# smu-ivpl/FastInterCU-VVC

Hardware: AMD Instinct MI355X
Metric: CU-inferences/sec (batch 4096, 128x128) (higher is better)
Workload: dtype f16 (fp32 accumulate)

## Files before the change

fastintercu-vvc_amd/csrc/mlt_dispatch.cpp:

```cpp
#include "mlt_runtime.h"

const char *tuning_env(const char *name) {
  const char *e = std::getenv("MLT_TUNING");
  return (e && e[0] == '1') ? std::getenv(name) : nullptr;
}

const Tuning &tuning() {
  static const Tuning t = [] {
    auto num = [](const char *name, long dflt) { const char *e = tuning_env(name); return e ? std::atol(e) : dflt; };
    auto on = [](const char *name) { return tuning_env(name) != nullptr; };
    auto cap = [&](const char *name) { const long v = num(name, 0); return (int)(v > 0 ? v : 256); };
    Tuning u{};
    u.debug_dump_dir = tuning_env("MLT_DEBUG_DUMP_DIR");
    u.xl_kill = (int)num("MLT_XL_KILL", 0); u.xl_kill_layer = (int)num("MLT_XL_KILL_LAYER", -1);
    u.lat_pixels = num("MLT_LAT_PIXELS", 16384L);
    u.no_exact_lat = on("MLT_NO_EXACT_LAT"); u.exact_patch_big = !on("MLT_EXACT_PATCH_64K");
    u.wg_cap = cap("MLT_WG_CAP"); u.wg_cap0 = cap("MLT_WG_CAP0"); u.wg_cap1 = cap("MLT_WG_CAP1"); u.wg_cap2 = cap("MLT_WG_CAP2");
    u.l0_mfma32 = on("MLT_L0_MFMA32"); u.l1_mfma32 = !on("MLT_L1_MFMA16");
    u.no_block_fusion = on("MLT_NO_BLOCK_FUSION");
    u.no_chain = on("MLT_NO_CHAIN") || u.no_block_fusion; u.no_chain_s2 = on("MLT_NO_CHAIN_S2"); u.no_c16 = on("MLT_NO_C16"); u.chain64 = !on("MLT_NO_CHAIN64");
    u.no_l0_s5 = on("MLT_NO_L0_S5");
    u.l0_stream_min = on("MLT_NO_L0_STREAM") ? 0 : (int)num("MLT_L0_STREAM_MIN", 128);
    u.l1_stream_min = on("MLT_NO_L1_STREAM") ? 0 : (int)num("MLT_L1_STREAM_MIN", 128);
    u.guard_wait_mode = on("MLT_GUARD_SPIN_WAIT") ? 1 : on("MLT_GUARD_BLOCKING_WAIT") ? 2 : 0;
    u.no_small_mix = on("MLT_NO_SMALL_MIX"); u.no_mag_guard = on("MLT_NO_MAG_GUARD");
    u.no_graph = on("MLT_NO_GRAPH") || u.debug_dump_dir != nullptr;
    return u;
  }();
  return t;
}

namespace {

int gap_slots(int hw) { return hw >= 32 ? hw / 32 : 1; }

size_t ws_per_cu(const mlt::Model &m, int S, bool some_exact = false) {
  const int h0 = S / 2 > 0 ? S / 2 : 1;
  const int planes = (m.exact || some_exact) ? 2 : 1;
  size_t b = 4 * ((size_t)h0 * h0 * 32 * 2 * planes + 256);
  int h = S;
  for (int s = 0; s < m.n_stages; ++s) {
    h = h / 2 > 0 ? h / 2 : 1;
    b += (size_t)h * h * m.planes[s] * 2 * planes + 256;
    if (s >= 1) b += (size_t)gap_slots(h * h) * m.planes[s] * 4 + 256;
  }
  return b + 4096;
}

int ensure_ws(mlt_ctx *ctx, size_t bytes) {
  if (bytes <= ctx->ws_bytes) return MLT_OK;
  if (ctx->ws) { HIP_TRY(ctx, hipStreamSynchronize(ctx->stream)); (void)hipFree(ctx->ws); ctx->ws = nullptr; ctx->ws_bytes = 0; }
  ++ctx->ws_gen;
  HIP_TRY(ctx, hipMalloc((void **)&ctx->ws, bytes));
  ctx->ws_bytes = bytes;
  return MLT_OK;
}
}
void release_ws(mlt_ctx *ctx) {
  if (ctx->ws) { (void)hipFree(ctx->ws); ctx->ws = nullptr; ctx->ws_bytes = 0; }
  ++ctx->ws_gen;
}
namespace {

int debug_dump(mlt_ctx *ctx, const char *name, const void *dptr, size_t bytes) {
  const char *dir = tuning().debug_dump_dir;
  static int seq = 0;
  if (!dir) return MLT_OK;
  std::vector<char> host(bytes);
  HIP_TRY(ctx, hipStreamSynchronize(ctx->stream));
  HIP_TRY(ctx, hipMemcpy(host.data(), dptr, bytes, hipMemcpyDeviceToHost));
  char path[1200];
  std::snprintf(path, sizeof path, "%s/%02d_%s.bin", dir, seq++, name);
  if (FILE *f = std::fopen(path, "wb")) { std::fwrite(host.data(), 1, bytes, f); std::fclose(f); }
  return MLT_OK;
}

// ... 220 lines not shown
  a.x = x; a.y = y; a.w1 = B.conv1.d_w; a.w2 = B.conv2.d_w; a.bias1 = B.conv1.d_bias; a.bias2 = B.conv2.d_bias;
  a.w1_lo_off = B.conv1.plane_halves * 2; a.w2_lo_off = B.conv2.plane_halves * 2; a.scale1 = B.conv1.acc_scale; a.scale2 = B.conv2.acc_scale;
  a.n = n; a.h_l = ilog2(h); a.ntiles = n * (h / (w2 ? 8 : 16)) * (h / 32);
  const int wg_cap = tuning().wg_cap;
  const int grid_x = a.ntiles > wg_cap ? wg_cap : a.ntiles;
  char name[48];
  std::snprintf(name, sizeof name, "block_s1_32_h%d(conv1+conv2)", h);
  const double px = (double)n * h * h;
  Launch L{ctx};
  hipEvent_t e0 = nullptr, e1 = nullptr;
  int rc = L.prof_begin(name, 2.0 * px * 32 * 32 * 9 * 2, px * 32 * 2 * 2 + 2.0 * 18 * 1024, e0, e1, w2 ? "hi+lo weights" : "single pass");
  if (rc) return rc;
  plan_note(ctx, {{"x", x}, {"y", y}}, {{"grid", grid_x}});
  LAUNCH_TRY(ctx, mlt_launch_block32(a, w2, grid_x, ctx->stream));
  if ((rc = L.prof_end(e1))) return rc;
  return debug_dump(ctx, name, y, (size_t)px * 32 * 2);
}

int run_chain3(mlt_ctx *ctx, const mlt::Block &B0, const mlt::Block &B1, int n, int h, const void *t, const void *sc, void *y, float *gap,
               const void *s2_in, bool x_c16, bool y_c16, void *b0_hbm, bool sc_c16) {
  const int c = B0.conv2.cout;
  ChainArgs a{};
  a.x = s2_in ? s2_in : t; a.nconv = 3; a.y = y; a.gap = gap; a.n = n; a.zero = ctx->zero_page;
  a.x_c16 = x_c16 ? 1 : 0; a.y_c16 = y_c16 ? 1 : 0; a.res0_c16 = sc_c16 ? 1 : 0;
  const mlt::PackedConv *pcs[3] = {&B0.conv2, &B1.conv1, &B1.conv2};
  const bool w2 = B0.conv2.w2;
  for (int k = 0; k < 3; ++k) {
    a.cv[k].w = pcs[k]->d_w; a.cv[k].bias = pcs[k]->d_bias; a.cv[k].acc_scale = pcs[k]->acc_scale; a.cv[k].relu = 1;
    a.cv[k].w_lo_off = pcs[k]->plane_halves * 2;
    a.cv[k].lo8_scale = 0x01010101 * ((127 - pcs[k]->lo8_exp) & 0xFF);
  }
  a.cv[0].res_mode = s2_in ? 2 : 1; a.cv[0].res = sc; a.cv[0].save = 1; a.cv[2].res_mode = 2;
  if (c == 64) {
    a.cv[0].save = 0; a.cv[0].y = b0_hbm; a.cv[2].res_mode = 1; a.cv[2].res = b0_hbm;
  }
  if (s2_in) {
    const mlt::PackedConv &p2 = B0.conv1_s2c;
    a.s2_w = p2.d_w; a.s2_bias = p2.d_bias; a.s2_bias_sc = p2.d_bias_sc; a.s2_scale = p2.acc_scale;
  }
  const int hw = h * h;
  a.gap_slots = gap_slots(hw); a.gap_l = hw >= 32 ? 5 : ilog2(hw);
  const int wg_cap = tuning().wg_cap;
  const int spw = c == 256 ? 2 : 1;
  const int ntiles = (n + spw - 1) / spw;
  const int grid_x = ntiles > wg_cap ? wg_cap : ntiles;
  char name[48];
  std::snprintf(name, sizeof name, s2_in ? "stage_%d_h%d(s2+sc,conv2,conv1,conv2)" : "chain3_s1_%d_h%d(conv2+conv1+conv2)", c, h);
  const double px = (double)n * hw;
  const double flops = 3.0 * 2.0 * px * c * c * 9 + (s2_in ? 2.0 * px * c * (c / 2) * 10 : 0.0);
  const double bytes = (s2_in ? px * 4 * (c / 2) * 2 : px * c * 2 * 2) + (y ? px * c * 2 : 0.0) + 3.0 * (double)B0.conv2.w.size() * 2 +
                       (s2_in ? (double)B0.conv1_s2c.w.size() * 2 : 0.0);
  Launch L{ctx};
  hipEvent_t e0 = nullptr, e1 = nullptr;
  char variant[96];
  std::snprintf(variant, sizeof variant, "%s%s%s%s%s", w2 ? "hi+lo weights" : "single pass", x_c16 ? ", x chunk-major" : "", sc_c16 ? ", sc chunk-major" : "", y_c16 ? ", y chunk-major" : "",
                gap ? ", GAP" : "");
  int rc = L.prof_begin(name, flops, bytes, e0, e1, variant);
  if (rc) return rc;
  plan_note(ctx, {{"x", a.x}, {"sc", s2_in ? nullptr : sc}, {"y", y}, {"gap", gap}, {"b0", c == 64 ? b0_hbm : nullptr}}, {{"grid", grid_x}});
  LAUNCH_TRY(ctx, mlt_launch_chain(c, h, s2_in != nullptr, ctx->lds_oob_zero, w2, a, grid_x, ctx->stream));
  if ((rc = L.prof_end(e1))) return rc;
  if (y && (rc = debug_dump(ctx, name, y, (size_t)px * c * 2))) return rc;
  return MLT_OK;
}

int run_layer1_stream(mlt_ctx *ctx, const mlt::Block &B0, const mlt::Block &B1, int n, const void *t, const void *sc, void *y, float *gap, bool y_c16) {
  Layer1Args a{};
  a.t = t; a.sc = sc; a.y = y; a.y_c16 = y_c16 ? 1 : 0; a.gap = gap; a.gap_slots = gap_slots(32 * 32); a.n = n;
  const mlt::PackedConv *pcs[3] = {&B0.conv2, &B1.conv1, &B1.conv2};
  for (int k = 0; k < 3; ++k) { a.w[k] = pcs[k]->d_w; a.bias[k] = pcs[k]->d_bias; a.scale[k] = pcs[k]->acc_scale; }
  const int wg_cap = tuning().wg_cap1;
  const int grid_x = n > wg_cap ? wg_cap : n;
  const double px = (double)n * 32 * 32;
  Launch L{ctx};
  hipEvent_t e0 = nullptr, e1 = nullptr;
  int rc = L.prof_begin("layer1_stream_h32(conv2+conv1+conv2)", 3.0 * 2.0 * px * 64 * 64 * 9, px * 64 * 2 * 3 + 3.0 * 72 * 1024, e0, e1, y_c16 ? "single pass, y chunk-major, GAP" : "single pass, GAP");
  if (rc) return rc;
  const bool mfma32 = tuning().l1_mfma32;
  plan_note(ctx, {{"t", t}, {"sc", sc}, {"y", y}, {"gap", gap}}, {{"grid", grid_x}});
  LAUNCH_TRY(ctx, mlt_launch_layer1_stream(a, mfma32, grid_x, ctx->stream));
  if ((rc = L.prof_end(e1))) return rc;
  return debug_dump(ctx, "chain3_s1_64_h32(conv2+conv1+conv2)", y, (size_t)px * 64 * 2);
}

enum : unsigned { CLS_QUADS = 1u, CLS_FLAT = 2u, CLS_L0_STREAM = 4u, CLS_L1_STREAM = 8u, CLS_CHAIN0 = 16u  };
unsigned batch_class(const NetCfg &c, int n, const Planes &pl, bool has_flat) {
  const Tuning &tn = tuning();
  unsigned cls = 0;
  if (pl.aligned8()) cls |= CLS_QUADS;
  if (has_flat) cls |= CLS_FLAT;
  if (tn.l0_stream_min > 0 && n >= tn.l0_stream_min) cls |= CLS_L0_STREAM;
  if (tn.l1_stream_min > 0 && n >= tn.l1_stream_min) cls |= CLS_L1_STREAM;
  for (int s = 1; s < c.m->n_stages; ++s) {
    const int h = c.h_in(s), ho = h / 2 > 0 ? h / 2 : 1;
    if ((long)n * ho * ho > tn.lat_pixels) cls |= CLS_CHAIN0 << s;
  }
  return cls;
}


NetPlan plan_network(const mlt_ctx *ctx, const NetCfg &c, unsigned cls) {
  const Tuning &tn = tuning();
  const mlt::Model &m = *c.m;
  NetPlan P;
  auto add = [&](PlanStep::Kind k, int s) -> PlanStep & { PlanStep st{}; st.kind = k; st.s = (int8_t)s; P.push_back(st); return P.back(); };
  auto wants_chain = [&](int s) -> bool {
    if (s <= 0 || s >= m.n_stages || tn.no_chain || !(cls & (CLS_CHAIN0 << s))) return false;
    const mlt::Model &mm = c.model_of(s, 1);
    if (mm.exact || (mm.w2 && !ctx->lds_oob_zero)) return false;
    const int h = c.h_in(s), ho = h / 2 > 0 ? h / 2 : 1;
    const mlt::PackedConv &c2 = mm.blocks[s][0].conv2;
    const bool packing_ok = (m.planes[s] == 64 ? (c2.ct == 64 && c2.gt == 9 && tn.chain64) : (c2.ct == 128 && c2.gt == 3)) && (!mm.w2 || c2.lo8 || m.planes[s] == 64);
    return mlt_chain_supported(m.planes[s], ho) && c2.taps == 9 && c2.kc == 64 && packing_ok;
// ... 239 lines not shown
```

fastintercu-vvc_amd/csrc/mlt_kernels.h:

```cpp
#pragma once
#include <hip/hip_runtime.h>
#include <stdint.h>

#define MLT_MAX_HEADS_K 4
#define MLT_MAX_LOGITS_K 16
#define MLT_FLAT_RANGE 6
#define MLT_FLAT_EXACT_SHIFT 16

struct ConvArgs {
  const void *x;
  void *y;
  const void *w;
  const float *bias;
  const void *res;
  const void *zero;
  int n;
  int ntiles;
  int hin_l, hout_l;
  int tw_l, th_l, spw_l;
  int ph, pw, rp, half;
  uint32_t pw_magic, ph_magic, rp_magic;
  int patch_bytes;
  int relu;
  int y_c16;
// ... 57 lines not shown
  const float *bias, *bias_sc, *bias2, *bias3, *bias4;
  void *y;
  int32_t *flat;
  float acc_scale;
  int n;
  const void *w5;
  const float *bias5, *bias5_sc;
  void *y_t, *y_sc;
  float scale5;
};

#define MLT_L1_LDS_BYTES 159008
struct Layer1Args {
  const void *t;
  const void *sc;
  const void *w[3];
  const float *bias[3];
  float scale[3];
  void *y;
  int y_c16;
  float *gap;
  int gap_slots, n;
};

struct ChainConv {
  const void *w;
  size_t w_lo_off;
  int lo8_scale;
  const float *bias;
  float acc_scale;
  int relu;
  int res_mode;
  int save;
  const void *res;
  void *y;
};
struct ChainArgs {
  const void *x;
  const void *s2_w;
  const float *s2_bias, *s2_bias_sc;
  float s2_scale;
  const void *zero;
  ChainConv cv[3];
  int nconv;
  void *y;
  int y_c16;
  int x_c16;
  int res0_c16;
  float *gap;
  int gap_slots, gap_l;
  int n;
};
hipError_t mlt_launch_chain(int c, int h, bool with_s2, bool oob_zero, bool w2, const ChainArgs &a, int grid_x, hipStream_t st);
bool mlt_chain_supported(int c, int h);
hipError_t mlt_probe_lds_oob(int *d_ok, hipStream_t st);
bool mlt_stage_supported(int c, int h);

struct DecisionRec {
  int32_t split_mode, raw_mode;
  float confidence, margin;
  int32_t level_mode[MLT_MAX_HEADS_K];
  float level_conf[MLT_MAX_HEADS_K];
};
#define MLT_CONF_BAND_FRAC 0.75f

#define MLT_MAX_CAND_K 6
struct CandRec {
  uint32_t mask;
  int32_t count;
  int8_t order[8];
  float prob[MLT_MAX_CAND_K];
};

struct HeadArgs {
  const float *gap[MLT_MAX_HEADS_K];
  int slots[MLT_MAX_HEADS_K];
  const float *w[MLT_MAX_HEADS_K];
  const float *b[MLT_MAX_HEADS_K];
  int c[MLT_MAX_HEADS_K], hw[MLT_MAX_HEADS_K], classes[MLT_MAX_HEADS_K];
  int n_heads, decision_head;
  const int32_t *poc, *qp;
  float *logits;
  int32_t *split;
  DecisionRec *dec;
  float min_conf, g_conf_band;
  CandRec *cand;
  float cand_cov, g_cand_band;
  int cand_max;
  int32_t *g_count, *g_idx, *g_flat;
  int g_flat_thr, g_near_thr;
  float g_margin;
  float *mag;
  float g_mag_thr;
  int32_t *g_next;
};

struct FlatStatArgs {
  const int16_t *org, *pred;
  long org_row_stride, org_cu_stride, pred_row_stride, pred_cu_stride;
  int32_t *flat;
  int n, s_l;
};
struct GuardSelectArgs {
  const int32_t *flat;
  const float *logits;
  int32_t *idx;
// ... 89 lines not shown
```

fastintercu-vvc_amd/csrc/mlt_kernels.hip:

```cpp
#include <hip/hip_runtime.h>
#include <hip/hip_fp16.h>
#include <stdint.h>

#include <atomic>
#include <utility>

#include "mlt_kernels.h"

#ifndef CFG_ASM_PIPE
#define CFG_ASM_PIPE 1
#endif
#ifndef CFG_S2_BIAS_EARLY
#define CFG_S2_BIAS_EARLY 1
#endif
#ifndef CFG_DMA_SPREAD
#define CFG_DMA_SPREAD 5
#endif
#ifndef CFG_RING_FD16
#define CFG_RING_FD16 1
#endif
#ifndef CFG_RING_RES_EARLY
#define CFG_RING_RES_EARLY 1
#endif
#ifndef CFG_BIAS_EARLY
// ... 138 lines not shown
  r = __builtin_amdgcn_cvt_scalef32_pk_fp8_f16(r, prep(h[1]), 1.0f, true);
  q = __builtin_amdgcn_cvt_scalef32_pk_fp8_f16(q, prep(h[2]), 1.0f, false);
  q = __builtin_amdgcn_cvt_scalef32_pk_fp8_f16(q, prep(h[3]), 1.0f, true);
  d0 = *(uint32_t *)&r;
  d1 = *(uint32_t *)&q;
}
__device__ __forceinline__ float16v mfma_xl8(const half8 &a_lo, const half8 &a_hi, const half8 &b_lo, const half8 &b_hi, const float16v &c, int scale_a, int scale_b) {
  int8v a, b;
  const uint32_t *pl = (const uint32_t *)&a_lo, *ph = (const uint32_t *)&a_hi, *ql = (const uint32_t *)&b_lo, *qh = (const uint32_t *)&b_hi;
#pragma unroll
  for (int e = 0; e < 4; ++e) { a[e] = (int)pl[e]; a[4 + e] = (int)ph[e]; b[e] = (int)ql[e]; b[4 + e] = (int)qh[e]; }
  return __builtin_amdgcn_mfma_scale_f32_32x32x64_f8f6f4(a, b, c, 0, 0, 0, scale_a, 0, scale_b);
}

typedef uint32_t uint4v __attribute__((ext_vector_type(4)));
__device__ __forceinline__ uint4v pair16(half4 qa, half4 qb) {
  uint32_t ax = ((uint32_t *)&qa)[0], ay = ((uint32_t *)&qa)[1], bx = ((uint32_t *)&qb)[0], by = ((uint32_t *)&qb)[1];
  auto r0 = __builtin_amdgcn_permlane32_swap(ax, bx, false, false);
  auto r1 = __builtin_amdgcn_permlane32_swap(ay, by, false, false);
  uint4v v;
  v[0] = r0[0]; v[1] = r1[0]; v[2] = r0[1]; v[3] = r1[1];
  return v;
}
__device__ __forceinline__ void unpair16(uint4v v, half4 &qa, half4 &qb) {
  auto r0 = __builtin_amdgcn_permlane32_swap(v[0], v[2], false, false);
  auto r1 = __builtin_amdgcn_permlane32_swap(v[1], v[3], false, false);
  ((uint32_t *)&qa)[0] = r0[0]; ((uint32_t *)&qa)[1] = r1[0];
  ((uint32_t *)&qb)[0] = r0[1]; ((uint32_t *)&qb)[1] = r1[1];
}

typedef float float2v __attribute__((ext_vector_type(2)));
template <int Q, class ACC = float16v> __device__ __forceinline__ half4 act_quad(const ACC &A, float scale, const float4v &b, bool has_res, const half4 &r, bool relu, float *x4 = nullptr) {
  half4 out;
#pragma unroll
  for (int ep = 0; ep < 2; ++ep) {
    float2v a2 = {A[4 * Q + 2 * ep], A[4 * Q + 2 * ep + 1]};
    const float2v b2 = {b[2 * ep], b[2 * ep + 1]};
    float2v x2 = a2 * scale + b2;
    if (has_res) {
      const float2v r2 = {(float)r[2 * ep], (float)r[2 * ep + 1]};
      x2 += r2;
    }
    if (x4) { x4[2 * ep] = x2[0]; x4[2 * ep + 1] = x2[1]; }
    half2v h2 = __builtin_convertvector(x2, half2v);
    if (relu) h2 = __builtin_elementwise_max(h2, (half2v){(_Float16)0, (_Float16)0});
    out[2 * ep] = h2[0];
    out[2 * ep + 1] = h2[1];
  }
  return out;
}

#include "mlt_conv_kernels.inc"
#include "mlt_chain_kernel.inc"
#include "mlt_front_kernels.inc"
#include "mlt_layer0_kernel.inc"
#include "mlt_layer1_kernel.inc"
#include "mlt_tail_kernels.inc"
#include "mlt_picture_kernels.inc"
#include "mlt_tree_kernels.inc"

struct DeviceOnce {
  std::atomic<uint64_t> mask[4] = {};
  bool need(int *dev) const {
    if (hipGetDevice(dev) != hipSuccess) *dev = 0;
    return !(mask[(*dev >> 6) & 3].load(std::memory_order_acquire) & (1ull << (*dev & 63)));
  }
  void done(int dev) { mask[(dev >> 6) & 3].fetch_or(1ull << (dev & 63), std::memory_order_release); }
};
template <class K> static hipError_t ensure_big_lds(K kern, DeviceOnce &once) {
  int dev = 0;
  if (!once.need(&dev)) return hipSuccess;
  hipError_t e = hipFuncSetAttribute((const void *)kern, hipFuncAttributeMaxDynamicSharedMemorySize, 160 * 1024);
  if (e == hipSuccess) once.done(dev);
  return e;
}
template <int CIN, int COUT, int STRIDE, int TAPS, bool SC, int KC, int NSPLIT, int WCB, int WPB, int WAVES_C, int WAVES_P, int GT, int RB, int UN, int MINW, bool DMA, int CBP = 0, bool KMAJ = false>
static hipError_t launch_conv_t(const ConvArgs &a, int grid_x, int extra_lds, hipStream_t st) {
  auto kern = conv_mfma_kernel<CIN, COUT, STRIDE, TAPS, SC, KC, NSPLIT, WCB, WPB, WAVES_C, WAVES_P, GT, RB, UN, MINW, DMA, CBP, KMAJ>;
  constexpr int CBT = WCB * WAVES_C;
  constexpr int TT = TAPS + (SC ? 1 : 0);
  constexpr int NBUF = (TT / GT) > 1 ? RB : 1;
  const int patch_lds = (DMA ? 2 : ((NSPLIT == 2 || NSPLIT == 6) ? 2 : 1)) * a.patch_bytes;
  const int patch8 = NSPLIT == 5 ? ((a.patch_bytes / (KC * 2 + 16) + 1) * (KC + 16) + 1023) / 1024 * 1024 : 0;
  const int lds = patch_lds + NBUF * ((NSPLIT == 2 || NSPLIT == 3 || NSPLIT == 6 ? 2 : 1) * GT * (KC / 16) * CBT * 1024 + (NSPLIT == 5 ? GT * CBT * 2048 : 0)) + patch8 + extra_lds;
  static DeviceOnce once;
  if (hipError_t e = ensure_big_lds(kern, once); e != hipSuccess) return e;
  if (lds > 160 * 1024) return hipErrorInvalidValue;
  dim3 grid(grid_x, COUT / (32 * CBT));
  hipLaunchKernelGGL(kern, grid, dim3(64 * WAVES_C * WAVES_P), lds, st, a);
  return hipGetLastError();
}

template <int CIN, int COUT, int STRIDE, bool SC, int KC, int WCB, int WPB, int WAVES_C, int WAVES_P, int GT, int RB, int UNP, int MINW, int NWL, int FD>
static hipError_t launch_ring_dma_t(const ConvArgs &a, int grid_x, hipStream_t st) {
  auto kern = conv_ring_dma_kernel<CIN, COUT, STRIDE, SC, KC, WCB, WPB, WAVES_C, WAVES_P, GT, RB, UNP, MINW, NWL, FD>;
  constexpr int CBT = WCB * WAVES_C, NW = WAVES_C * WAVES_P;
  constexpr int NWP = NWL ? NWL - NWL / 2 : NW - NW / 2;
  const int lds = 2 * a.patch_bytes + RB * GT * (KC / 16) * CBT * 1024 + (NWL ? 32 * CBT * 4 * (SC ? 2 : 1) : 0);
  static DeviceOnce once;
  if (hipError_t e = ensure_big_lds(kern, once); e != hipSuccess) return e;
  if (lds > 160 * 1024 || (a.patch_bytes >> 10) > UNP * NWP) return hipErrorInvalidValue;
  dim3 grid(grid_x, COUT / (32 * CBT));
  hipLaunchKernelGGL(kern, grid, dim3(64 * (NW + NWL)), lds, st, a);
  return hipGetLastError();
}

// ... 332 lines not shown
#ifndef CFG_CHAIN_FD
#define CFG_CHAIN_FD 2
#endif
#ifndef CFG_CHAIN_SPLIT
#define CFG_CHAIN_SPLIT 1
#endif
#ifndef CFG_CHAINW2_RB
#define CFG_CHAINW2_RB 3
#endif
template <class K> static hipError_t launch_chain_t(K kern, DeviceOnce &once, const ChainArgs &a, int grid_x, int threads, int lds, hipStream_t st) {
  if (hipError_t e = ensure_big_lds(kern, once); e != hipSuccess) return e;
  hipLaunchKernelGGL(kern, dim3(grid_x), dim3(threads), lds, st, a);
  return hipGetLastError();
}
hipError_t mlt_launch_chain(int c, int h, bool with_s2, bool oob_zero, bool w2, const ChainArgs &a, int grid_x, hipStream_t st) {
  static_assert(CFG_BIG_GT == 3 && CFG_BIG_WCB == 2 && CFG_BIG_WC == 2, "chain_kernel reads the packing of the stand-alone 128->128 / 256->256 layers");
  constexpr int lds = 64 * 1024 + 2 * (CFG_BIG_GT * 4 * 4 * 1024);
  static DeviceOnce once[13];
  if (w2) {
    if (!oob_zero || with_s2 || a.nconv != 3) return hipErrorInvalidValue;
    if (c == 64 && h == 32)
      return launch_chain_t(chain_kernel<64, 5, 0, 2, 4, 1, 8, 1, 2, 1, 2, 3, true, false, false, true, true, false>, once[10], a, grid_x, 512, 128 * 1024 + 2 * 16 * 1024, st);
    if (c == 128 && h == 16)
      return launch_chain_t(chain_kernel<128, 4, 0, 2, 2, 2, 4, 1, 2, 1, 2, 3, true, false, true, true, true, true>, once[11], a, grid_x, 512, (64 + 2 * 24 + 32) * 1024, st);
    if (c == 256 && h == 8)
      return launch_chain_t(chain_kernel<256, 3, 1, 2, 1, 2, 4, 1, 2, 1, 2, 3, true, false, true, true, true, true>, once[12], a, grid_x, 512, (64 + 2 * 24 + 32) * 1024, st);
    return hipErrorInvalidValue;
  }
  if (c == 64 && h == 32 && a.nconv == 3 && !with_s2) {
    static_assert(CFG_64_WCB == 2 && CFG_64_WC == 1 && CFG_64_GT == 9, "chain_kernel<64,...> reads the packing of the stand-alone 64->64 layer");
    constexpr int RB64 = CFG_CHAIN64_GT == 1 ? 4 : 2, lds64 = 128 * 1024 + 4 * 8 * 1024;
    if (oob_zero) return launch_chain_t(chain_kernel<64, 5, 0, 2, 4, 1, 8, CFG_CHAIN64_GT, RB64, 1, 2, 3, true, false, false, true>, once[6], a, grid_x, 512, lds64, st);
    return launch_chain_t(chain_kernel<64, 5, 0, 2, 4, 1, 8, CFG_CHAIN64_GT, RB64, 1, 2, 3, true, false, false, false>, once[7], a, grid_x, 512, lds64, st);
  }
  if (c == 128 && h == 16) {
    if (with_s2 && a.nconv == 3) {
      if (oob_zero) return launch_chain_t(chain_kernel<128, 4, 0, 2, 2, 2, 4, 3, 2, CFG_CHAIN_FD, 2, 3, true, true, true, true>, once[4], a, grid_x, 512, lds, st);
      return launch_chain_t(chain_kernel<128, 4, 0, 2, 2, 2, 4, 3, 2, CFG_CHAIN_FD, 2, 3, true, true, true, false>, once[8], a, grid_x, 512, lds, st);
    }
    if (a.nconv == 3) return launch_chain_t(chain_kernel<128, 4, 0, 2, 2, 2, 4, 3, 2, CFG_CHAIN_FD, 2, 3, CFG_CHAIN_SPLIT != 0>, once[0], a, grid_x, 512, lds, st);
    if (a.nconv == 2) return launch_chain_t(chain_kernel<128, 4, 0, 2, 2, 2, 4, 3, 2, CFG_CHAIN_FD, 2, 2, CFG_CHAIN_SPLIT != 0>, once[1], a, grid_x, 512, lds, st);
  }
  if (c == 256 && h == 8) {
    if (with_s2 && a.nconv == 3) {
      if (oob_zero) return launch_chain_t(chain_kernel<256, 3, 1, 2, 1, 2, 4, 3, 2, CFG_CHAIN_FD, 2, 3, true, true, true, true>, once[5], a, grid_x, 512, lds, st);
      return launch_chain_t(chain_kernel<256, 3, 1, 2, 1, 2, 4, 3, 2, CFG_CHAIN_FD, 2, 3, true, true, true, false>, once[9], a, grid_x, 512, lds, st);
    }
    if (a.nconv == 3) return launch_chain_t(chain_kernel<256, 3, 1, 2, 1, 2, 4, 3, 2, CFG_CHAIN_FD, 2, 3, CFG_CHAIN_SPLIT != 0>, once[2], a, grid_x, 512, lds, st);
    if (a.nconv == 2) return launch_chain_t(chain_kernel<256, 3, 1, 2, 1, 2, 4, 3, 2, CFG_CHAIN_FD, 2, 2, CFG_CHAIN_SPLIT != 0>, once[3], a, grid_x, 512, lds, st);
  }
  return hipErrorInvalidValue;
}

hipError_t mlt_launch_stem5(const Stem5Args &a, int nsplit, int grid_x, int lds, hipStream_t st) {
  if (nsplit == 3) hipLaunchKernelGGL(stem5_kernel<3>, dim3(grid_x), dim3(256), lds, st, a);
  else if (nsplit == 2) hipLaunchKernelGGL(stem5_kernel<2>, dim3(grid_x), dim3(256), lds, st, a);
  else hipLaunchKernelGGL(stem5_kernel<1>, dim3(grid_x), dim3(256), lds, st, a);
  return hipGetLastError();
}

hipError_t mlt_launch_block32(const Block32Args &a, bool w2, int grid_x, hipStream_t st) {
  static DeviceOnce once[2];
  if (w2) {
    constexpr int lds = (12 * 36 + 10 * 34) * 80 + 4 * 18 * 1024;
    if (hipError_t e = ensure_big_lds(block32_kernel<3, true>, once[1]); e != hipSuccess) return e;
    hipLaunchKernelGGL((block32_kernel<3, true>), dim3(grid_x), dim3(512), lds, st, a);
    return hipGetLastError();
  }
  constexpr int lds = (20 * 36 + 18 * 34) * 80 + 2 * 18 * 1024;
  if (hipError_t e = ensure_big_lds(block32_kernel<4, false>, once[0]); e != hipSuccess) return e;
  hipLaunchKernelGGL((block32_kernel<4, false>), dim3(grid_x), dim3(512), lds, st, a);
  return hipGetLastError();
}

hipError_t mlt_launch_stem_block(const StemBlockArgs &a, bool w2, int grid_x, hipStream_t st) {
  constexpr int lds = 3 * (39 * 72 * 4 + 16) + 2 * (18 * 34 * 80) + 18 * 1024 + 256 + 2 * 1024;
  static DeviceOnce once[2];
  if (w2) {
    if (hipError_t e = ensure_big_lds(stem_block_kernel<true>, once[1]); e != hipSuccess) return e;
    hipLaunchKernelGGL(stem_block_kernel<true>, dim3(grid_x), dim3(128 * CFG_SB_NWS), lds + 2 * 1024, st, a);
    return hipGetLastError();
  }
  if (hipError_t e = ensure_big_lds(stem_block_kernel<false>, once[0]); e != hipSuccess) return e;
  hipLaunchKernelGGL(stem_block_kernel<false>, dim3(grid_x), dim3(128 * CFG_SB_NWS), lds, st, a);
  return hipGetLastError();
}

template <bool F5, bool M16> static hipError_t launch_layer0_stream_t(const Layer0Args &a, int grid_x, hipStream_t st) {
  static DeviceOnce once;
  if (hipError_t e = ensure_big_lds(layer0_stream_kernel<F5, M16>, once); e != hipSuccess) return e;
  hipLaunchKernelGGL((layer0_stream_kernel<F5, M16>), dim3(grid_x), dim3(1024), F5 ? MLT_L0F_LDS_BYTES : MLT_L0_LDS_BYTES, st, a);
  return hipGetLastError();
}
hipError_t mlt_launch_layer0_stream(const Layer0Args &a, bool fuse5, bool mfma32, int grid_x, hipStream_t st) {
  if (fuse5) return mfma32 ? launch_layer0_stream_t<true, false>(a, grid_x, st) : launch_layer0_stream_t<true, true>(a, grid_x, st);
  return launch_layer0_stream_t<false, false>(a, grid_x, st);
}

hipError_t mlt_launch_layer1_stream(const Layer1Args &a, bool mfma32, int grid_x, hipStream_t st) {
  static DeviceOnce once[2];
  if (mfma32) {
    if (hipError_t e = ensure_big_lds(layer1_stream_kernel<false>, once[0]); e != hipSuccess) return e;
    hipLaunchKernelGGL(layer1_stream_kernel<false>, dim3(grid_x), dim3(1024), MLT_L1_LDS_BYTES, st, a);
    return hipGetLastError();
  }
  if (hipError_t e = ensure_big_lds(layer1_stream_kernel<true>, once[1]); e != hipSuccess) return e;
// ... 53 lines not shown
```

fastintercu-vvc_amd/csrc/mlt_runtime.h:

```cpp
#pragma once
#include <hip/hip_runtime.h>

#include <chrono>
#include <cmath>
#include <cstddef>
#include <cstdio>
#include <cstdlib>
#include <cstring>
#include <map>
#include <tuple>
#include <mutex>
#include <string>
#include <thread>
#include <vector>

#include "../../include/mltcnn.h"
#include "mlt_kernels.h"
#include "mlt_model.h"
#include "mlt_tier_search.h"

const char *tuning_env(const char *name);

struct Tuning {
  const char *debug_dump_dir;
  int xl_kill, xl_kill_layer;
  long lat_pixels;
  bool no_exact_lat;
  bool exact_patch_big;
  int wg_cap, wg_cap0, wg_cap1, wg_cap2;
  bool l0_mfma32, l1_mfma32;
  bool no_chain, no_chain_s2, no_c16, chain64, no_block_fusion, no_l0_s5;
  int l0_stream_min, l1_stream_min;
  int guard_wait_mode;
  bool no_small_mix, no_mag_guard, no_graph;
};
const Tuning &tuning();

inline int size_index(int size) {
  switch (size) {
    case 128: return 0;
    case 64: return 1;
    case 32: return 2;
    case 16: return 3;
    default: return -1;
  }
}
inline int ilog2(int v) { int l = 0; while ((1 << l) < v) ++l; return l; }

struct NetCfg {
  int S = 0;
  mlt::Model *m = nullptr, *mback = nullptr, *mx = nullptr;
  unsigned back_mask = 0, x_units = 0;
  mlt::Model &model_of(int s, int u) const { return ((x_units >> (2 * s + u)) & 1u) ? *mx : (mback && ((back_mask >> (2 * s + u)) & 1u)) ? *mback : *m; }
  int h_in(int s) const { int h = S; for (int i = 0; i < s; ++i) h = h / 2 > 0 ? h / 2 : 1; return h; }
};

struct PlanStep {
  enum Kind : uint8_t {
    FLAT_STAT,
    LAYER0_STREAM,
    STEM_BLOCK,
    STEM5,
    CONV_S2,
    CHAIN,
    LAYER1_STREAM,
    CONV_B0C2,
    BLOCK32,
    CONV_B1C1,
    CONV_B1C2,
    HEADS
  } kind;
  int8_t s = 0;
  bool front = false;
  bool inside_s2 = false;
  bool x_c16 = false;
  bool sc_c16 = false;
  bool y_c16 = false;
};
using NetPlan = std::vector<PlanStep>;
using PlanKey = std::tuple<const void *, const void *, const void *, unsigned, unsigned, unsigned>;

struct SizeState {
  bool enabled = false, loaded = false;
  std::map<PlanKey, NetPlan> plans;
  bool exact = false;
// ... 243 lines not shown
```

Measured before the change: 1.048 million.

## Add direct-to-register weight streaming kernel for the 256-channel 8x8 stage

Adds a dedicated kernel for the c=256, h=8 stage (stride-2 entry, shortcut and three 3x3 convs). It streams weight fragments from global memory straight into registers through a rolling prefetch queue, so only activations and input patches are staged in LDS. It also prefetches the next tile's input patches during the epilogues. The kernel is selected when the batch is at least 257 and the LDS out-of-bounds-zero probe passes, and it replaces the generic chain kernel there. The cost is more register pressure and a lot of new hand-scheduled code that depends on exact waitcnt ordering.

```diff
diff --git a/fastintercu-vvc_amd/csrc/mlt_dispatch.cpp b/fastintercu-vvc_amd/csrc/mlt_dispatch.cpp
--- a/fastintercu-vvc_amd/csrc/mlt_dispatch.cpp
+++ b/fastintercu-vvc_amd/csrc/mlt_dispatch.cpp
@@ -22,6 +22,7 @@
     u.no_l0_s5 = on("MLT_NO_L0_S5");
     u.l0_stream_min = on("MLT_NO_L0_STREAM") ? 0 : (int)num("MLT_L0_STREAM_MIN", 128);
     u.l1_stream_min = on("MLT_NO_L1_STREAM") ? 0 : (int)num("MLT_L1_STREAM_MIN", 128);
+    u.s3_direct_min = on("MLT_NO_S3_DIRECT") ? 0 : (int)num("MLT_S3_DIRECT_MIN", MLT_S3_DIRECT_MIN_DEFAULT);
     u.guard_wait_mode = on("MLT_GUARD_SPIN_WAIT") ? 1 : on("MLT_GUARD_BLOCKING_WAIT") ? 2 : 0;
     u.no_small_mix = on("MLT_NO_SMALL_MIX"); u.no_mag_guard = on("MLT_NO_MAG_GUARD");
     u.no_graph = on("MLT_NO_GRAPH") || u.debug_dump_dir != nullptr;
@@ -348,13 +349,16 @@
                        (s2_in ? (double)B0.conv1_s2c.w.size() * 2 : 0.0);
   Launch L{ctx};
   hipEvent_t e0 = nullptr, e1 = nullptr;
-  char variant[96];
-  std::snprintf(variant, sizeof variant, "%s%s%s%s%s", w2 ? "hi+lo weights" : "single pass", x_c16 ? ", x chunk-major" : "", sc_c16 ? ", sc chunk-major" : "", y_c16 ? ", y chunk-major" : "",
-                gap ? ", GAP" : "");
+  const int s3_min = tuning().s3_direct_min;
+  const bool direct = c == 256 && h == 8 && s2_in && !w2 && ctx->lds_oob_zero && s3_min > 0 && n >= s3_min;
+  char variant[112];
+  std::snprintf(variant, sizeof variant, "%s%s%s%s%s%s", w2 ? "hi+lo weights" : "single pass", direct ? ", weights to registers" : "", x_c16 ? ", x chunk-major" : "",
+                sc_c16 ? ", sc chunk-major" : "", y_c16 ? ", y chunk-major" : "", gap ? ", GAP" : "");
   int rc = L.prof_begin(name, flops, bytes, e0, e1, variant);
   if (rc) return rc;
   plan_note(ctx, {{"x", a.x}, {"sc", s2_in ? nullptr : sc}, {"y", y}, {"gap", gap}, {"b0", c == 64 ? b0_hbm : nullptr}}, {{"grid", grid_x}});
-  LAUNCH_TRY(ctx, mlt_launch_chain(c, h, s2_in != nullptr, ctx->lds_oob_zero, w2, a, grid_x, ctx->stream));
+  if (direct) LAUNCH_TRY(ctx, mlt_launch_stage256_direct(a, grid_x, ctx->stream));
+  else LAUNCH_TRY(ctx, mlt_launch_chain(c, h, s2_in != nullptr, ctx->lds_oob_zero, w2, a, grid_x, ctx->stream));
   if ((rc = L.prof_end(e1))) return rc;
   if (y && (rc = debug_dump(ctx, name, y, (size_t)px * c * 2))) return rc;
   return MLT_OK;
diff --git a/fastintercu-vvc_amd/csrc/mlt_kernels.h b/fastintercu-vvc_amd/csrc/mlt_kernels.h
--- a/fastintercu-vvc_amd/csrc/mlt_kernels.h
+++ b/fastintercu-vvc_amd/csrc/mlt_kernels.h
@@ -133,6 +133,8 @@
   int n;
 };
 hipError_t mlt_launch_chain(int c, int h, bool with_s2, bool oob_zero, bool w2, const ChainArgs &a, int grid_x, hipStream_t st);
+#define MLT_S3_DIRECT_MIN_DEFAULT 257
+hipError_t mlt_launch_stage256_direct(const ChainArgs &a, int grid_x, hipStream_t st);
 bool mlt_chain_supported(int c, int h);
 hipError_t mlt_probe_lds_oob(int *d_ok, hipStream_t st);
 bool mlt_stage_supported(int c, int h);
diff --git a/fastintercu-vvc_amd/csrc/mlt_kernels.hip b/fastintercu-vvc_amd/csrc/mlt_kernels.hip
--- a/fastintercu-vvc_amd/csrc/mlt_kernels.hip
+++ b/fastintercu-vvc_amd/csrc/mlt_kernels.hip
@@ -214,6 +214,7 @@
 
 #include "mlt_conv_kernels.inc"
 #include "mlt_chain_kernel.inc"
+#include "mlt_stage256_kernel.inc"
 #include "mlt_front_kernels.inc"
 #include "mlt_layer0_kernel.inc"
 #include "mlt_layer1_kernel.inc"
@@ -652,6 +653,12 @@
   return hipErrorInvalidValue;
 }
 
+hipError_t mlt_launch_stage256_direct(const ChainArgs &a, int grid_x, hipStream_t st) {
+  static DeviceOnce once;
+  if (a.nconv != 3 || !a.s2_w) return hipErrorInvalidValue;
+  return launch_chain_t(stage256_direct_kernel, once, a, grid_x, 512, 160 * 1024, st);
+}
+
 hipError_t mlt_launch_stem5(const Stem5Args &a, int nsplit, int grid_x, int lds, hipStream_t st) {
   if (nsplit == 3) hipLaunchKernelGGL(stem5_kernel<3>, dim3(grid_x), dim3(256), lds, st, a);
   else if (nsplit == 2) hipLaunchKernelGGL(stem5_kernel<2>, dim3(grid_x), dim3(256), lds, st, a);
diff --git a/fastintercu-vvc_amd/csrc/mlt_runtime.h b/fastintercu-vvc_amd/csrc/mlt_runtime.h
--- a/fastintercu-vvc_amd/csrc/mlt_runtime.h
+++ b/fastintercu-vvc_amd/csrc/mlt_runtime.h
@@ -31,6 +31,7 @@
   bool l0_mfma32, l1_mfma32;
   bool no_chain, no_chain_s2, no_c16, chain64, no_block_fusion, no_l0_s5;
   int l0_stream_min, l1_stream_min;
+  int s3_direct_min;
   int guard_wait_mode;
   bool no_small_mix, no_mag_guard, no_graph;
 };
diff --git a/fastintercu-vvc_amd/csrc/mlt_stage256_kernel.inc b/fastintercu-vvc_amd/csrc/mlt_stage256_kernel.inc
--- /dev/null
+++ b/fastintercu-vvc_amd/csrc/mlt_stage256_kernel.inc
@@ -0,0 +1,312 @@
+#ifndef CFG_S3D_FD
+#define CFG_S3D_FD 2
+#endif
+#ifndef CFG_S3D_FDS
+#define CFG_S3D_FDS 1
+#endif
+__global__ __launch_bounds__(512, 2) void stage256_direct_kernel(const ChainArgs a) {
+  constexpr int C = 256, HL = 3, H = 8, HW = 64, M = 128, KC = 64, NCHUNK = 4, KS = 4, SLOTS = 8, TAPS = 9, NW = 8;
+  constexpr int REGION = M * KC * 2, ACT = NCHUNK * REGION;
+  constexpr int AD = 8, FD = CFG_S3D_FD, FDS = CFG_S3D_FDS;
+  constexpr int CHB = 2, NB1 = CHB * TAPS * KS;
+  constexpr int NI1 = NCHUNK * TAPS * KS;
+  constexpr int CIN = C / 2, HIN = 2 * H, KCS = 16, NCS = CIN / KCS, TAPS_S = 10;
+  constexpr int CHS = 4, NBS = CHS * TAPS_S, NIS = NCS * TAPS_S;
+  constexpr int PRS = 2 * H + 1, PCW = 2 * H + 1, PPS = PRS * PCW, PPIX = PPS * 2;
+  constexpr int PBYTES = (PPIX * KCS * 2 + 1023) / 1024 * 1024, PPIECE = PBYTES / 1024, PPW = (PPIECE + NW - 1) / NW;
+  constexpr int NP_HI = 5;
+  constexpr size_t WPASS1 = (size_t)NCHUNK * TAPS * KS * 4 * 1024, WPASS_S = (size_t)NCS * TAPS_S * 4 * 1024;
+  static_assert(NB1 % AD == 0 && NBS % AD == 0 && NI1 % NB1 == 0 && NIS % NBS == 0, "a body starts at A slot 0");
+  static_assert(ACT + NP_HI * PBYTES <= 160 * 1024 && (NCS - NP_HI) * PBYTES <= ACT, "LDS layout of the patches");
+  static_assert(FD >= 1 && FD * 4 <= 15 && FDS >= 1 && FDS <= FD, "lgkmcnt is 4 bits; the B fragment registers are sized for FD");
+
+  extern __shared__ __attribute__((aligned(16))) char smem[];
+  const uint32_t lds0 = (uint32_t)(uintptr_t)LDS_PTR(smem);
+  const int tid = threadIdx.x, lane = tid & 63;
+  const int w = __builtin_amdgcn_readfirstlane(tid >> 6);
+  const int ps = w >> 2, i4 = w & 3, ib = w & 1;
+  const int p = lane & 31, h = lane >> 5;
+  const int lane16 = lane * 16;
+
+  const int pr = p < 4 ? p : p < 12 ? p + 12 : p < 16 ? p - 8 : p < 20 ? p + 8 : p < 28 ? p - 12 : p;
+  int mj[4], pj[4];
+#pragma unroll
+  for (int j = 0; j < 4; ++j) {
+    mj[j] = j * 32 + pr;
+    const int q = mj[j] >> 3, k = q & 7;
+    pj[j] = ((q & ~7) | ((k & 1) << 2) | (k >> 1)) * 8 + (mj[j] & 7);
+  }
+  auto swz = [](int q) { return ((q >> 1) & (SLOTS - 1)) ^ (((q >> 5) & 1) << 2); };
+
+  const int ntiles = (a.n + 1) >> 1;
+  int t = blockIdx.x;
+  const int tstep = gridDim.x;
+  if (t >= ntiles) return;
+
+  uint32_t pvo[PPW];
+#pragma unroll
+  for (int k = 0; k < PPW; ++k) {
+    const int piece = w + k * NW;
+    const int it = piece * 64 + lane, qS = it >> 1, pos = it & 1;
+    const int sl = pos ^ ((qS >> 3) & 1);
+    const int sm = qS / PPS, rem = qS - sm * PPS, r = rem / PCW, kk = rem - r * PCW;
+    const int ri = r - 1, ci = kk <= H ? 2 * kk - 1 : 2 * (kk - H - 1);
+    const bool live = qS < PPIX && ri >= 0 && ri < HIN && ci >= 0 && ci < HIN;
+    const uint32_t off = a.x_c16 ? ((ri * HIN + ci) * KCS + sl * 8) * 2 : ((ri * HIN + ci) * CIN + sl * 8) * 2;
+    pvo[k] = live ? off | ((uint32_t)sm << 30) : 0x80000000u;
+  }
+  const uint32_t chunk_stride = a.x_c16 ? HIN * HIN * KCS * 2 : KCS * 2;
+  auto poff = [](int chunk) { return chunk < NP_HI ? ACT + chunk * PBYTES : (chunk - NP_HI) * PBYTES; };
+  auto patch_dma = [&](int tile, int chunk) {
+    char *dst = smem + poff(chunk);
+    const char *xb = (const char *)a.x + (size_t)chunk * chunk_stride;
+    uint32_t zo = ((int)blockIdx.x * 64 * NW + tid) * 16;
+    asm volatile("" : "+v"(zo));
+    const char *zsrc = (const char *)a.zero + (zo & 0xFFF0);
+#pragma unroll
+    for (int k = 0; k < PPW; ++k) {
+      const int piece = w + k * NW;
+      if (piece >= PPIECE) break;
+      uint32_t v = pvo[k];
+      asm volatile("" : "+v"(v));
+      int n = (tile << 1) + (int)((v >> 30) & 1);
+      n = n < a.n ? n : a.n - 1;
+      const char *src = (int)v < 0 ? zsrc : xb + (size_t)n * (size_t)(CIN * HIN * HIN * 2) + (v & 0x3FFFFFFFu);
+      glds16(src, dst + piece * 1024);
+    }
+  };
+
+#pragma unroll 1
+  for (int c = 0; c < NCS; ++c) patch_dma(t, c);
+  float pb_cv[3], pb_t, pb_sc;
+  {
+    const int bo = (w & ~1) * 32 + lane;
+#pragma unroll
+    for (int c = 0; c < 3; ++c) pb_cv[c] = a.cv[c].bias[bo];
+    pb_t = a.s2_bias[bo];
+    pb_sc = a.s2_bias_sc[bo];
+#pragma unroll
+    for (int c = 0; c < 3; ++c) asm volatile("" : "+v"(pb_cv[c]));
+    asm volatile("" : "+v"(pb_t), "+v"(pb_sc));
+  }
+  const int pb_lane = 16 * h;
+  auto bias_rows = [&](float v, float4v(&out)[4]) {
+    int base = pb_lane + ib * 128;
+    asm volatile("" : "+v"(v), "+v"(base));
+#pragma unroll
+    for (int q = 0; q < 4; ++q)
+#pragma unroll
+      for (int e = 0; e < 4; ++e) out[q][e] = __builtin_bit_cast(float, __builtin_amdgcn_ds_bpermute(base + (8 * q + e) * 4, __builtin_bit_cast(int, v)));
+  };
+
+  half8 fa[AD];
+  const char *ap;
+  auto set_seg = [&](int seg) {
+    const char *b = seg == 0   ? (const char *)KARG(const void *, s2_w) + ps * WPASS_S
+                    : seg == 1 ? (const char *)KARG(const void *, cv[0].w) + ps * WPASS1
+                    : seg == 2 ? (const char *)KARG(const void *, cv[1].w) + ps * WPASS1
+                               : (const char *)KARG(const void *, cv[2].w) + ps * WPASS1;
+    ap = b + i4 * 1024 + lane16;
+  };
+  set_seg(0);
+  auto issue_a = [&](auto sc) {
+    constexpr int s = decltype(sc)::value;
+    asm volatile("global_load_dwordx4 %0, %1, off" : "=v"(fa[s]) : "v"(ap) : "memory");
+    ap += 4096;
+  };
+  static_for<AD - 1>([&](auto sc) { issue_a(sc); });
+
+  uint4v keep[4][2];
+#pragma unroll
+  for (int j = 0; j < 4; ++j)
+#pragma unroll
+    for (int qq = 0; qq < 2; ++qq) keep[j][qq] = uint4v{0u, 0u, 0u, 0u};
+
+  for (; t < ntiles; t += tstep) {
+#pragma unroll
+    for (int j = 0; j < 4; ++j) asm volatile("" : "+v"(pj[j]));
+    const bool has_next = t + tstep < ntiles;
+    asm volatile("s_waitcnt vmcnt(0)\n\ts_barrier" ::: "memory");
+
+    float16v acc[4];
+    half8 fb[FD + 1][4];
+    {
+      float16v accs[4];
+#pragma unroll
+      for (int j = 0; j < 4; ++j)
+#pragma unroll
+        for (int r = 0; r < 16; ++r) { acc[j][r] = 0.f; accs[j][r] = 0.f; }
+#pragma unroll 1
+      for (int cb = 0; cb < NCS / CHS; ++cb) {
+        int bS[4];
+        uint32_t pbk = 0;
+        auto issue_b = [&](auto ic) {
+          constexpr int it = decltype(ic)::value, sl = it % (FDS + 1), c = it / TAPS_S, tt = it % TAPS_S;
+          constexpr int te = tt == 9 ? 4 : tt, dy = te / 3, dx = te % 3;
+          constexpr int off = dy * PCW + (dx == 1 ? H + 1 : dx / 2);
+          if constexpr (tt == 0) {
+            pbk = lds0 + poff(cb * CHS + c);
+#pragma unroll
+            for (int j = 0; j < 4; ++j) {
+              asm volatile("" : "+v"(pj[j]));
+              bS[j] = ((pj[j] >> (2 * HL)) * PRS + 2 * ((pj[j] >> HL) & (H - 1))) * PCW + (pj[j] & (H - 1));
+            }
+          }
+          static_for<4>([&](auto jj) {
+            constexpr int j = decltype(jj)::value;
+            const int qS = bS[j] + off;
+            lds_read128<0>(fb[sl][j], pbk + qS * (KCS * 2) + ((h ^ ((qS >> 3) & 1)) << 4));
+          });
+        };
+        static_for<(FDS < NBS ? FDS : NBS)>([&](auto ic) { issue_b(ic); });
+        static_for<NBS>([&](auto ic) {
+          constexpr int it = decltype(ic)::value, sl = it % (FDS + 1), tt = it % TAPS_S;
+          if constexpr (it + AD - 1 == NBS) {
+            if (cb == NCS / CHS - 1) set_seg(1);
+          }
+          issue_a(std::integral_constant<int, (it + AD - 1) % AD>{});
+          if constexpr (it + FDS < NBS) issue_b(std::integral_constant<int, it + FDS>{});
+          asm volatile("s_waitcnt vmcnt(%0)" ::"n"(AD - 1) : "memory");
+          lds_wait<(NBS - 1 - it < FDS ? NBS - 1 - it : FDS) * 4>();
+          lds_touch(fa[it % AD]);
+#pragma unroll
+          for (int j = 0; j < 4; ++j) lds_touch(fb[sl][j]);
+#pragma unroll
+          for (int j = 0; j < 4; ++j) {
+            if constexpr (tt == 9) accs[j] = __builtin_amdgcn_mfma_f32_32x32x16_f16(fa[it % AD], fb[sl][j], accs[j], 0, 0, 0);
+            else acc[j] = __builtin_amdgcn_mfma_f32_32x32x16_f16(fa[it % AD], fb[sl][j], acc[j], 0, 0, 0);
+          }
+        });
+      }
+      asm volatile("s_barrier" ::: "memory");
+      if (has_next) {
+#pragma unroll 1
+        for (int c = 0; c < NP_HI; ++c) patch_dma(t + tstep, c);
+      }
+      float4v b1[4], bs[4];
+      const float s2_scale = KARG(float, s2_scale);
+      bias_rows(pb_t, b1);
+      bias_rows(pb_sc, bs);
+#pragma unroll
+      for (int j = 0; j < 4; ++j)
+        static_for<2>([&](auto qc) {
+          constexpr int qq = decltype(qc)::value;
+          half4 ht[2], hc[2];
+          const half4 none{};
+          ht[0] = act_quad<2 * qq>(acc[j], s2_scale, b1[2 * qq], false, none, true);
+          ht[1] = act_quad<2 * qq + 1>(acc[j], s2_scale, b1[2 * qq + 1], false, none, true);
+          hc[0] = act_quad<2 * qq>(accs[j], s2_scale, bs[2 * qq], false, none, false);
+          hc[1] = act_quad<2 * qq + 1>(accs[j], s2_scale, bs[2 * qq + 1], false, none, false);
+          keep[j][qq] = pair16(hc[0], hc[1]);
+          const uint4v wt = pair16(ht[0], ht[1]);
+          const int cb = w * 32 + 16 * qq + 8 * h;
+          *(uint4v *)(smem + (cb / KC) * REGION + pj[j] * (KC * 2) + ((((cb % KC) / 8) ^ swz(pj[j])) << 4)) = wt;
+        });
+      asm volatile("s_waitcnt lgkmcnt(0)\n\ts_barrier" ::: "memory");
+    }
+
+#pragma unroll 1
+    for (int cvi = 0; cvi < 3; ++cvi) {
+#pragma unroll
+      for (int j = 0; j < 4; ++j)
+#pragma unroll
+        for (int r = 0; r < 16; ++r) acc[j][r] = 0.f;
+#pragma unroll 1
+      for (int cb = 0; cb < NCHUNK / CHB; ++cb) {
+        const uint32_t plb = lds0 + cb * (CHB * REGION);
+        uint32_t rowa[4], hs[4];
+        auto issue_b = [&](auto ic) {
+          constexpr int it = decltype(ic)::value, sl = it % (FD + 1), c = it / (TAPS * KS), tap = (it / KS) % TAPS, ks = it % KS;
+          constexpr int dy = tap / 3, dx = tap % 3;
+          if constexpr (ks == 0) {
+#pragma unroll
+            for (int j = 0; j < 4; ++j) {
+              if constexpr (tap == 0) asm volatile("" : "+v"(pj[j]));
+              const int yy = ((pj[j] >> HL) & (H - 1)) + dy - 1, xx = (pj[j] & (H - 1)) + dx - 1;
+              const bool ok = (unsigned)yy < (unsigned)H && (unsigned)xx < (unsigned)H;
+              const int q = ok ? pj[j] + (dy - 1) * H + (dx - 1) : pj[j];
+              rowa[j] = ok ? plb + q * (KC * 2) : 0x100000u;
+              hs[j] = (h * 16) ^ (swz(q) << 4);
+            }
+          }
+          static_for<4>([&](auto jj) {
+            constexpr int j = decltype(jj)::value;
+            lds_read128<c * REGION>(fb[sl][j], rowa[j] + (hs[j] ^ (ks * 32)));
+          });
+        };
+        static_for<FD>([&](auto ic) { issue_b(ic); });
+        static_for<NB1>([&](auto ic) {
+          constexpr int it = decltype(ic)::value, sl = it % (FD + 1);
+          if constexpr (it + AD - 1 == NB1) {
+            if (cb == NCHUNK / CHB - 1) set_seg(cvi == 2 ? 0 : cvi + 2);
+          }
+          issue_a(std::integral_constant<int, (it + AD - 1) % AD>{});
+          if constexpr (it + FD < NB1) issue_b(std::integral_constant<int, it + FD>{});
+          asm volatile("s_waitcnt vmcnt(%0)" ::"n"(AD - 1) : "memory");
+          lds_wait<(NB1 - 1 - it < FD ? NB1 - 1 - it : FD) * 4>();
+          lds_touch(fa[it % AD]);
+#pragma unroll
+          for (int j = 0; j < 4; ++j) lds_touch(fb[sl][j]);
+#pragma unroll
+          for (int j = 0; j < 4; ++j) acc[j] = __builtin_amdgcn_mfma_f32_32x32x16_f16(fa[it % AD], fb[sl][j], acc[j], 0, 0, 0);
+        });
+      }
+      asm volatile("s_barrier" ::: "memory");
+      if (cvi < 2) {
+        auto epi = [&](auto cc) {
+          constexpr int cv = decltype(cc)::value;
+          constexpr bool RES = cv == 0;
+          float4v bi[4];
+          bias_rows(pb_cv[cv], bi);
+          const float sc_cv = KARG(float, cv[cv].acc_scale);
+#pragma unroll
+          for (int j = 0; j < 4; ++j)
+            static_for<2>([&](auto qc) {
+              constexpr int qq = decltype(qc)::value;
+              half4 ra{}, rb{}, hq[2];
+              if constexpr (RES) unpair16(keep[j][qq], ra, rb);
+              hq[0] = act_quad<2 * qq>(acc[j], sc_cv, bi[2 * qq], RES, ra, true);
+              hq[1] = act_quad<2 * qq + 1>(acc[j], sc_cv, bi[2 * qq + 1], RES, rb, true);
+              const uint4v wv = pair16(hq[0], hq[1]);
+              if constexpr (RES) keep[j][qq] = wv;
+              const int cb = w * 32 + 16 * qq + 8 * h;
+              *(uint4v *)(smem + (cb / KC) * REGION + pj[j] * (KC * 2) + ((((cb % KC) / 8) ^ swz(pj[j])) << 4)) = wv;
+            });
+        };
+        if (cvi == 0) epi(std::integral_constant<int, 0>{});
+        else epi(std::integral_constant<int, 1>{});
+        asm volatile("s_waitcnt lgkmcnt(0)\n\ts_barrier" ::: "memory");
+      } else {
+        if (has_next) {
+#pragma unroll 1
+          for (int c = NP_HI; c < NCS; ++c) patch_dma(t + tstep, c);
+        }
+#pragma unroll
+        for (int j = 0; j < 4; ++j) asm volatile("" : "+v"(pj[j]), "+v"(mj[j]));
+        int opix[4], gidx[4];
+        const int gslots = KARG(int, gap_slots), nall = KARG(int, n);
+#pragma unroll
+        for (int j = 0; j < 4; ++j) {
+          const int nn = (t << 1) + (pj[j] >> (2 * HL));
+          const bool ok = nn < nall;
+          opix[j] = ok ? nn * HW + (pj[j] & (HW - 1)) : -1;
+          gidx[j] = ok ? nn * gslots + ((mj[j] & (HW - 1)) >> 5) : -1;
+        }
+        float4v bq[1][4], bsq[1][4];
+        bias_rows(pb_cv[2], bq[0]);
+        ConvArgs ea{};
+        ea.y = KARG(void *, y); ea.gap = KARG(float *, gap); ea.gap_slots = KARG(int, gap_slots); ea.gap_l = KARG(int, gap_l);
+        ea.acc_scale = KARG(float, cv[2].acc_scale); ea.relu = 1;
+        ea.y_c16 = KARG(int, y_c16); ea.hout_l = HL;
+        ea.res = (const void *)smem;
+        float16v acc_sc[1][1];
+        uint4v resl[1][1][2];
+        int he = h, pe = p;
+        asm volatile("" : "+v"(he), "+v"(pe));
+        conv_epilogue<C, 128, 1, 4, false, 1>(ea, ps, i4, he, pe, opix, gidx, reinterpret_cast<float16v(&)[1][4]>(acc), acc_sc, bq, bsq,
+                                              reinterpret_cast<const uint4v(&)[1][4][2]>(keep), resl);
+      }
+    }
+  }
+  asm volatile("s_waitcnt vmcnt(0)" ::: "memory");
+}
```

Result: no change. 1.039 million (-0.9%).
